# zhuzhui-2000/mobilesuperresolution

Measured on AMD Instinct MI355X. Metric: HR megapixels/sec (WDSR-B x4, 48x48 LR patches), full training step, higher is better.
Workload: dtype bf16; 1 GPU; WDSR-B x4, 16 blocks / 24 units, 48x48 LR patches, batch 32 per GPU, fwd+L1+bwd+Adam; global_batch=32, parallelism=dp1

## Files before the change

include/sr_hotpath.h:

```cpp
#ifndef SR_HOTPATH_H
#define SR_HOTPATH_H
#include <stddef.h>
#include <stdint.h>

#ifdef __cplusplus
extern "C" {
#endif

typedef void* sr_stream_t;

#define SR_DTYPE_F32 0
#define SR_DTYPE_BF16 1

int sr_abi_version(void);

int sr_wdsr_block_fwd(const void* x, void* y, const void* wblob, const float* cinit,
                      int N, int H, int W, int F, int dtype, sr_stream_t stream);

int sr_wdsr_block2_fwd(const void* x, void* ya, void* yb, const void* wblob_a, const void* wblob_b,
                       const float* cinit_a, const float* cinit_b, void* tsave_a, void* tsave_b, int N, int H, int W,
                       int F, int dtype, sr_stream_t stream);

int sr_wdsr_block2_bwd_data(const void* xa, const void* xb, const void* dyb, void* dxb, void* dxa,
                            const void* wblob_a, const void* wblob_b, const float* cinit_a, const float* cinit_b,
// ... 154 lines not shown
typedef struct { const int* idx; void* out; long src_off, src_stride; int n, reps, as_float; } sr_pack_seg_t;
typedef struct { const float* partial; const int* sidx; const int* dst; long dst_off, dst_stride, slab; int wgs, n, reps; } sr_unpack_seg_t;
int sr_param_pack(const float* flat, float* src, const int* chan_tab, int n_chan, const int* bias_tab, const float* bias_const,
                  int n_bias, const sr_pack_seg_t* segs, int nseg, int dtype, sr_stream_t stream);
int sr_param_grads(const float* flat, float* dsrc, float* gflat, const int* chan_tab, int n_chan, const int* bias_tab,
                   int n_bias, const sr_unpack_seg_t* segs, int nseg, sr_stream_t stream);

typedef struct {
  int F, NB, R, dtype, N, H, W;
  float mean;
  const float* flat; float* gflat;
  const int* chan_tab; int n_chan;
  const int* bias_tab; const float* bias_const; int n_bias;
  float* src; float* dsrc;
  long src_head_off, src_body_off, src_body_stride, src_tail_off;
  const int* idx_head; int n_idx_head;
  const int* idx_body; int n_idx_body;
  const int* idx_cinit; int n_idx_cinit;
  const int* idx_tail; int n_idx_tail;
  void* blob_head; void* blob_body; float* cinit_body; void* blob_tail;
  float* part_a; float* part_b; float* part_tail; float* part_head;
  int wgs_body, wgs_tail, wgs_head;
  int slab_a, slab_b, slab_tail, slab_head;
  const int* ga_sidx; const int* ga_dst; int n_ga;
  const int* gb_sidx; const int* gb_dst; int n_gb;
  const int* gt_sidx; const int* gt_dst; int n_gt;
  const int* gh_sidx; const int* gh_dst; int n_gh;
  const float* x; void* acts; void* grads; float* out; const float* dout;
  void* tsave; void* dtsave;
  const float* hr; int loss_kind; float loss_gscale; float* loss_part;
  int nb_split, chan_split, bias_split;
  int adam_in_wn_bwd;
  int one_block32;
} sr_wdsr_net_t;

#define SR_NET_SAVE_ACTS 1
#define SR_NET_WEIGHTS_PACKED 2
#define SR_NET_PACK_ONLY 4
#define SR_NET_SKIP_TAIL 8
int sr_wdsr_net_forward(const sr_wdsr_net_t* net, int flags, sr_stream_t stream);
int sr_wdsr_net_backward(const sr_wdsr_net_t* net, sr_stream_t stream);
int sr_wdsr_net_backward_part(const sr_wdsr_net_t* net, int part, sr_stream_t stream);

int sr_pixel_shuffle(const float* in, float* out, int N, int C, int H, int W, int r, int inverse, sr_stream_t stream);

int sr_tail_bwd_loss(const float* sr, const float* hr, int loss_kind, float gscale, float* loss_part, const void* feat,
                     const float* x_nchw, float mean, const void* wblob, void* dfeat, float* partial, int wgs, int N, int H,
                     int W, int F, int R, int dtype, sr_stream_t stream);

int sr_tail_train(const float* hr, int loss_kind, float gscale, float* loss_part, const void* feat, const float* x_nchw, float mean,
                  const void* wblob, void* dfeat, float* partial, int wgs, int N, int H, int W, int F, int R, int dtype,
                  sr_stream_t stream);

typedef struct { float w_lerp, beta2, one_minus_beta2, bc2_sqrt, eps, neg_step_size; } sr_adam_t;
int sr_adam_step(float* param, const float* grad, float* exp_avg, float* exp_avg_sq, long n, const sr_adam_t* a,
                 const float* loss_part, int n_loss, float loss_scale, float* loss_out, sr_stream_t stream);
int sr_loss_value(const float* loss_part, int n_loss, float loss_scale, float* loss_out, sr_stream_t stream);
int sr_scale_by(void* y, const void* x, long n, const float* scale, int dtype, sr_stream_t stream);
int sr_wdsr_net_train_step(const sr_wdsr_net_t* net, float* exp_avg, float* exp_avg_sq, long n_params, const sr_adam_t* a,
                           float loss_scale, float* loss_out, sr_stream_t stream);

int sr_conv7_fwd(const void* x, const void* wpacked, const float* bias, void* y, int N, int H, int W, int CIN, int COUT, int relu,
                 int out_f32, sr_stream_t stream);

int sr_probe_mfma_bf16(const void* a_frag, const void* b_frag, float* acc_out, sr_stream_t stream);
int sr_probe_mfma_f32(const float* a_frag, const float* b_frag, float* acc_out, sr_stream_t stream);
int sr_probe_tr_read(const void* img_bf16, int n_elems, const int* lane_elem_off, void* out_bf16x4,
                     sr_stream_t stream);
int sr_probe_copy(const void* src, void* dst, size_t n_bytes, sr_stream_t stream);
int sr_probe_launch_floor(void* out, int gx, int gy, int threads, int lds_bytes, int reps, sr_stream_t stream);
int sr_probe_launch_floor_graph(void* out, int gx, int gy, int threads, int lds_bytes, int reps, int iters,
                                float* us_per_launch, float* host_us_per_graph );
// ... 7 lines not shown
```

mobilesuperresolution_amd/_lib.py:

```python
from __future__ import annotations

import ctypes
import os
from ctypes import c_int, c_size_t, c_void_p

import torch

_HERE = os.path.dirname(os.path.abspath(__file__))
LIB_PATH = os.environ.get("SR_HOTPATH_LIB_PATH") or os.path.join(
    _HERE, "libsr_hotpath_dbg.so" if os.environ.get("SR_HOTPATH_DEBUG_LIB") == "1" else "libsr_hotpath.so")
ABI_VERSION = 19
DTYPE_CODE = {torch.float32: 0, torch.bfloat16: 1}
_HOT_DTYPES = {"fp32": torch.float32, "float32": torch.float32, "bf16": torch.bfloat16, "bfloat16": torch.bfloat16}


def hot_dtype(name=None) -> torch.dtype:
    name = name or os.environ.get("SR_HOT_DTYPE", "fp32")
    return name if isinstance(name, torch.dtype) else _HOT_DTYPES[str(name).lower()]


_P, _I, _Z, _L, _F = c_void_p, c_int, c_size_t, ctypes.c_long, ctypes.c_float
SIGNATURES = {
    "sr_abi_version": ([], _I),
    "sr_wdsr_block_fwd": ([_P, _P, _P, _P, _I, _I, _I, _I, _I, _P], _I),
    "sr_wdsr_block2_fwd": ([_P] * 9 + [_I] * 5 + [_P], _I),
    "sr_wdsr_fwd_rs": ([_P] * 9 + [_I] * 6 + [_P], _I),
    "sr_conv7_fwd": ([_P] * 4 + [_I] * 7 + [_P], _I),
    "sr_wdsr_fwd_rs_repeat": ([_P] * 9 + [_I] * 7 + [_P], _I),
    "sr_wdsr_block_wgrad_saved": ([_P] * 8 + [_I] * 7 + [_L] * 5 + [_P], _I),
    "sr_wdsr_block2_bwd_data": ([_P] * 11 + [_I] * 5 + [_P], _I),
    "sr_wdsr_block2_fwd_repeat": ([_P] * 7 + [_I] * 6 + [_P], _I),
    "sr_probe_launch_floor": ([_P, _I, _I, _I, _I, _I, _P], _I),
    "sr_probe_launch_floor_graph": ([_P, _I, _I, _I, _I, _I, _I, _P, _P], _I),
    "sr_debug_set_stamps": ([_P, _L], _I),
    "sr_c3_trunk_fwd": ([_P] * 6 + [_I] * 7 + [_L, _P], _I),
    "sr_c3_trunk_bwd": ([_P] * 11 + [_I] * 8 + [_L, _P], _I),
    "sr_c64_trunk_fwd": ([_P] * 7 + [_I] * 7 + [_L, _P], _I),
    "sr_c64_recon_fwd": ([_P, _P, _I, _P, _L, _P, _P, _P, _P, _P, _P, _P, _L] + [_I] * 5 + [_P], _I),
    "sr_mv_recon_fwd": ([_P, _P, _I, _P, _L, _L, _P, _P, _L, _L, _P] + [_I] * 5 + [_P], _I),
    "sr_mv_recon_bwd": ([_P, _P, _P, _P, _L, _L, _P, _P, _P, _P, _I, _P] + [_I] * 6 + [_P], _I),
    "sr_mv_recon_slab": ([], _I),
    "sr_tail_bwd": ([_P, _P, _P, _F, _P, _P, _P] + [_I] * 7 + [_P], _I),
    "sr_nas_dw_wgrad": ([_P, _P, _P, _P, _I, _I, _I, _I, _I, _I, _P], _I),
    "sr_wdsr_block_fwd_repeat": ([_P, _P, _P, _P, _I, _I, _I, _I, _I, _I, _P], _I),
# ... 31 lines not shown
    "sr_scale_by": ([_P, _P, _L, _P, _I, _P], _I),
    "sr_wdsr_net_train_step": ([_P, _P, _P, _L, _P, _F, _P, _P], _I),
    "sr_wdsr_net_forward": ([_P, _I, _P], _I),
    "sr_wdsr_net_backward": ([_P, _P], _I),
    "sr_wdsr_net_backward_part": ([_P, _I, _P], _I),
    "sr_probe_mfma_bf16": ([_P, _P, _P, _P], _I),
    "sr_probe_mfma_f32": ([_P, _P, _P, _P], _I),
    "sr_probe_tr_read": ([_P, _I, _P, _P, _P], _I),
    "sr_probe_copy": ([_P, _P, _Z, _P], _I),
    "sr_rm_block_fwd": ([_P] * 5 + [_I] * 6 + [_P], _I),
    "sr_rm_block_bwd_data": ([_P] * 4 + [_I] * 6 + [_P], _I),
    "sr_rm_wgrad": ([_P] * 4 + [_I] * 8 + [_P], _I),
    "sr_rm_tail_fwd": ([_P] * 3 + [_I] * 7 + [_P], _I),
    "sr_rm_unshuffle": ([_P, _P] + [_I] * 5 + [_P], _I),
    "sr_rm_tail_bwd_data": ([_P] * 3 + [_I] * 7 + [_P], _I),
}

class WdsrNet(ctypes.Structure):
    _fields_ = (
        [(n, _I) for n in ("F", "NB", "R", "dtype", "N", "H", "W")] + [("mean", _F)] +
        [("flat", _P), ("gflat", _P), ("chan_tab", _P), ("n_chan", _I),
         ("bias_tab", _P), ("bias_const", _P), ("n_bias", _I), ("src", _P), ("dsrc", _P)] +
        [(n, _L) for n in ("src_head_off", "src_body_off", "src_body_stride", "src_tail_off")] +
        [("idx_head", _P), ("n_idx_head", _I), ("idx_body", _P), ("n_idx_body", _I),
         ("idx_cinit", _P), ("n_idx_cinit", _I), ("idx_tail", _P), ("n_idx_tail", _I),
         ("blob_head", _P), ("blob_body", _P), ("cinit_body", _P), ("blob_tail", _P),
         ("part_a", _P), ("part_b", _P), ("part_tail", _P), ("part_head", _P)] +
        [(n, _I) for n in ("wgs_body", "wgs_tail", "wgs_head", "slab_a", "slab_b", "slab_tail", "slab_head")] +
        [("ga_sidx", _P), ("ga_dst", _P), ("n_ga", _I), ("gb_sidx", _P), ("gb_dst", _P), ("n_gb", _I),
         ("gt_sidx", _P), ("gt_dst", _P), ("n_gt", _I), ("gh_sidx", _P), ("gh_dst", _P), ("n_gh", _I),
         ("x", _P), ("acts", _P), ("grads", _P), ("out", _P), ("dout", _P), ("tsave", _P), ("dtsave", _P),
         ("hr", _P), ("loss_kind", _I), ("loss_gscale", _F), ("loss_part", _P),
         ("nb_split", _I), ("chan_split", _I), ("bias_split", _I), ("adam_in_wn_bwd", _I),
         ("one_block32", _I)])


class C3Warp(ctypes.Structure):
    _fields_ = [("frame", _P), ("frame_bs", _L), ("state", _P), ("flow", _P), ("flow_bs", _L), ("flow_bound", _P),
                ("dstate", _P), ("dflow", _P), ("dflow_bs", _L), ("x0_save", _P)]


class C3Unpack(ctypes.Structure):
    _fields_ = [("sidx0", _P), ("dst0", _P), ("n0", _I), ("sidx1", _P), ("dst1", _P), ("n1", _I), ("gflat", _P)]


class PackSeg(ctypes.Structure):
    _fields_ = [("idx", _P), ("out", _P), ("src_off", _L), ("src_stride", _L), ("n", _I), ("reps", _I), ("as_float", _I)]


class UnpackSeg(ctypes.Structure):
    _fields_ = [("partial", _P), ("sidx", _P), ("dst", _P), ("dst_off", _L), ("dst_stride", _L), ("slab", _L), ("wgs", _I),
                ("n", _I), ("reps", _I)]


class AdamScalars(ctypes.Structure):
    _fields_ = [(n, _F) for n in ("w_lerp", "beta2", "one_minus_beta2", "bc2_sqrt", "eps", "neg_step_size")]


_lib = None


class HotpathError(RuntimeError):
    pass


def _declare(lib):
    for name, (args, res) in SIGNATURES.items():
# ... 92 lines not shown
```

mobilesuperresolution_amd/csrc/sr_abi.hip:

```cpp
#include <algorithm>
#include "../../include/sr_hotpath.h"
#include "wdsr_block.h"
#include "wdsr_fwd_rs.h"
#include "wdsr_fwd_stream.h"
#include "wdsr_bwd_rs.h"
#include "wdsr_bwd_pair_lds.h"
#include "wdsr_wgrad_rs.h"
#include "wdsr_ends.h"
#include "wdsr_prep.h"
#include "conv3x3.h"
#include "conv64.h"
#include "vsr_recon.h"
#include "mv_recon.h"
#include "spynet_conv.h"
#include "nas_block.h"
#include "nas_dw_lc.h"
#include "nas_bwd_fused.h"
#include "flow_warp.h"
#include "metrics.h"
#include "patches.h"
#include "clips.h"
#include "train_step.h"
#include "pixel_shuffle.h"
#include "result_block.h"

extern "C" int sr_abi_version(void) { return 19; }

namespace {

template <int F_, int E_, int L_>
struct WdsrDimsOf {
  static constexpr int F = F_, E = E_, L = L_;
  typedef BlockCfg<F_, E_, L_> Cfg;
};
template <int F> struct WdsrDims;
template <> struct WdsrDims<24> : WdsrDimsOf<24, 144, 20> {};
template <> struct WdsrDims<32> : WdsrDimsOf<32, 192, 26> {};

template <typename Fn>
int dispatch_f(int F, Fn&& fn) {
  if (F == 24) return fn(WdsrDims<24>{});
  if (F == 32) return fn(WdsrDims<32>{});
  return -1;
}
template <typename Fn>
int dispatch_ft(int F, int dtype, Fn&& fn) {
  return dispatch_f(F, [&](auto d) {
    if (dtype == SR_DTYPE_BF16) return fn(d, __bf16{});
    if (dtype == SR_DTYPE_F32) return fn(d, float{});
    return -1;
  });
}

struct Tiles { int x, y; };
template <typename C = WdsrDims<24>::Cfg>
Tiles block_tiles(int H, int W) {
  return Tiles{(W + C::TW - 1) / C::TW, (H + C::TH - 1) / C::TH};
}

// ... 948 lines not shown
    else if (F == 32) hipLaunchKernelGGL((nas_dw_wgrad3_kernel<32>), dim3(wgs), dim3(768), 0, st, (const __bf16*)yin, (const __bf16*)GZ, dwp, partial, N, H, W, tx, tpi, vs);
    else return -1;
    SR_HIP_CHECK_LAUNCH();
    return 0;
  }
#define CALL(T, F_) { typedef NasCfg<F_> C; const int tx = (W + C::TW - 1) / C::TW, tpi = tx * ((H + C::TH - 1) / C::TH); \
    hipLaunchKernelGGL((nas_dw_wgrad_kernel<T, F_>), dim3(wgs, 3), dim3(768), 0, st, (const T*)yin, (const T*)GZ, dwp, partial, N, H, W, tx, tpi, vs); }
  SR_NAS_DISPATCH_F32(CALL)
#undef CALL
  SR_HIP_CHECK_LAUNCH();
  return 0;
}

namespace {
template <typename T> int net_pack(const sr_wdsr_net_t* n, hipStream_t st) {
  const int cb = (n->n_chan + 3) / 4, bb = (n->n_bias + 255) / 256;
  hipLaunchKernelGGL(wn_src_kernel, dim3(cb + bb), dim3(256), 0, st, n->flat, n->src, (const int4*)n->chan_tab,
                     n->n_chan, n->bias_tab, n->bias_const, n->n_bias, cb);
  PackSegs ps;
  ps.nseg = 4;
  int blk = 0;
  auto add = [&](int k, const int* idx, void* out, long off, long stride, int cnt, int reps, int as_float) {
    ps.s[k] = PackSeg{idx, out, off, stride, cnt, reps, as_float, blk};
    blk += reps * ((cnt + 255) / 256);
  };
  add(0, n->idx_head, n->blob_head, n->src_head_off, 0, n->n_idx_head, 1, 0);
  add(1, n->idx_body, n->blob_body, n->src_body_off, n->src_body_stride, n->n_idx_body, n->NB, 0);
  add(2, n->idx_cinit, n->cinit_body, n->src_body_off, n->src_body_stride, n->n_idx_cinit, n->NB, 1);
  add(3, n->idx_tail, n->blob_tail, n->src_tail_off, 0, n->n_idx_tail, 1, 0);
  hipLaunchKernelGGL((pack_all_kernel<T>), dim3(blk), dim3(256), 0, st, n->src, ps);
  SR_HIP_CHECK_LAUNCH();
  return 0;
}
}

static bool net_saves_side_images(const sr_wdsr_net_t* n, bool backward) {
  return (n->F == 24 || n->F == 32) && n->dtype == SR_DTYPE_BF16 && n->tsave && (!backward || n->dtsave);
}
static long net_tiles(const sr_wdsr_net_t* n) {
  const Tiles t = block_tiles(n->H, n->W);
  return (long)n->N * t.x * t.y;
}
static bool net_uses_pairs(const sr_wdsr_net_t* n) {
  return n->dtype == SR_DTYPE_BF16 && net_tiles(n) <= 384 && (n->F == 24 || (n->F == 32 && !n->one_block32));
}
static bool net_step_fuses_tail(const sr_wdsr_net_t* n) {
  return n->dtype == SR_DTYPE_BF16 && n->R == 4 && (n->F == 24 || n->F == 32) && n->hr && n->N <= 65535;
}
static size_t side_image_bytes(const sr_wdsr_net_t* n) {
  typedef WdsrDims<24>::Cfg C;
  const Tiles t = block_tiles<C>(n->H, n->W);
  const int lp = n->F == 24 ? C::LP : WdsrDims<32>::Cfg::LP;
  return (size_t)n->N * ((size_t)t.x * t.y) * C::TH * C::TW * lp * 2;
}
struct NetView {
  const sr_wdsr_net_t* n;
  bool keeps_side;
  size_t esz = n->dtype == SR_DTYPE_BF16 ? 2 : 4;
  size_t act_bytes = (size_t)n->N * n->H * n->W * n->F * esz, blob_bytes = (size_t)n->n_idx_body * esz;
  size_t side_bytes = side_image_bytes(n);
  char* act(int i) const { return (char*)n->acts + (size_t)i * act_bytes; }
  char* grad(int i) const { return (char*)n->grads + (size_t)i * act_bytes; }
  char* blob(int i) const { return (char*)n->blob_body + (size_t)i * blob_bytes; }
  const float* cinit(int i) const { return n->cinit_body + (size_t)i * n->n_idx_cinit; }
  char* tsave(int i) const { return keeps_side ? (char*)n->tsave + (size_t)i * side_bytes : nullptr; }
  char* dtsave(int i) const { return keeps_side ? (char*)n->dtsave + (size_t)i * side_bytes : nullptr; }
};

extern "C" int sr_wdsr_net_forward(const sr_wdsr_net_t* n, int flags, sr_stream_t stream) {
  if (!n || !n->flat || !n->src) return -2;
  if (!(flags & SR_NET_PACK_ONLY) && (!n->x || !n->acts || !n->out)) return -2;
  hipStream_t st = (hipStream_t)stream;
  const int save_acts = flags & SR_NET_SAVE_ACTS;
  int rc = 0;
  if (!(flags & SR_NET_WEIGHTS_PACKED)) rc = n->dtype == SR_DTYPE_BF16 ? net_pack<__bf16>(n, st) : net_pack<float>(n, st);
  if (rc || (flags & SR_NET_PACK_ONLY)) return rc;
  const NetView v{n, save_acts && net_saves_side_images(n, false)};
  char* acts = v.act(0);
  if ((rc = sr_head_fwd(n->x, acts, n->blob_head, n->mean, n->N, n->H, n->W, n->F, n->dtype, stream))) return rc;
  char* cur = acts;
  const bool pairs = net_uses_pairs(n) || (n->F == 24 && n->dtype == SR_DTYPE_BF16 &&
                                           ((!save_acts && net_tiles(n) >= 768) || fwd_stream_applies(n->N, n->H, n->W)));
  for (int i = 0, nb; i < n->NB; i += nb) {
    nb = pairs && i + 1 < n->NB ? 2 : 1;
    char* nxt = save_acts ? v.act(i + nb) : (cur == acts ? v.act(1) : acts);
    if (nb == 2)
      rc = sr_wdsr_block2_fwd(cur, save_acts ? v.act(i + 1) : nullptr, nxt, v.blob(i), v.blob(i + 1), v.cinit(i), v.cinit(i + 1),
                              v.tsave(i), v.tsave(i + 1), n->N, n->H, n->W, n->F, n->dtype, stream);
    else if (pairs)
      rc = sr_wdsr_fwd_rs(cur, nullptr, nxt, v.blob(i), nullptr, v.cinit(i), nullptr, v.tsave(i), nullptr, 1, n->N, n->H, n->W, n->F,
                          n->dtype, stream);
    else if (v.keeps_side)
      rc = dispatch_f(n->F, [&](auto d) {
        return launch_block_fwd<__bf16, decltype(d)::F>(cur, nxt, v.blob(i), v.cinit(i), n->N, n->H, n->W, st, v.tsave(i));
      });
    else
      rc = sr_wdsr_block_fwd(cur, nxt, v.blob(i), v.cinit(i), n->N, n->H, n->W, n->F, n->dtype, stream);
    if (rc) return rc;
    cur = nxt;
  }
  if (flags & SR_NET_SKIP_TAIL) return 0;
  return sr_tail_fwd(cur, n->x, n->out, n->blob_tail, n->mean, n->N, n->H, n->W, n->F, n->R, n->dtype, stream);
}

namespace {
struct FusedAdam { float* m; float* v; AdamArgs a; const float* loss_part; int n_loss; float loss_scale; float* loss_out; };
}
static int net_backward_part_impl(const sr_wdsr_net_t* n, int part, sr_stream_t stream, const FusedAdam* fa, bool tail_train = false) {
  if (!n || !n->flat || !n->gflat || !n->dsrc || !n->x || !n->acts || !n->grads || part < 0 || part > 2) return -2;
  if (tail_train && (part != 0 || !n->hr)) return -2;
  if (part != 2 && (n->hr ? ((!n->out && !tail_train) || !n->loss_part || (n->loss_kind != 1 && n->loss_kind != 2)) : !n->dout)) return -2;
  hipStream_t st = (hipStream_t)stream;
// ... 620 lines not shown
```

mobilesuperresolution_amd/csrc/wdsr_ends.h:

```cpp
#pragma once
#include "wdsr_block.h"

template <int F_, int R_>
struct EndsCfg {
  static constexpr int F = F_, R = R_;
  static constexpr int CO = 3 * R * R, NT = (CO + 31) / 32, COP = (CO + 7) / 8 * 8, CC = COP / 8, FC = F / 8;
  static constexpr int KST = (9 * FC + 15 + 1) / 2, KSTB = (9 * CC + 1) / 2;
  static constexpr int TH = 12, TW = 24, HW = TW + 2, HH = TH + 2, NPXH = HW * HH, NPXH_PAD = (NPXH + 31) / 32 * 32;
  static constexpr int NPT_O = (TH / 4) * (TW / 8), NPXC = TH * TW;
  static constexpr int FT_ELEMS = (NPXH_PAD + 2) * F;
  static constexpr int DC_ELEMS = (NPXH_PAD + 2) * COP;
  static constexpr int DCC_ELEMS = (NPXC + 2) * COP;
  static constexpr int DYC_ELEMS = (NPXC + 2) * F;
  template <int P> struct Img {
    static constexpr int IW = TW + 2 * P, IH = TH + 2 * P, NPI = IW * IH, ELEMS = (NPI + 8) * 4;
  };
  static constexpr int TAIL_TILES = 14 * NT;
};

template <typename T> SR_DEV typename FragOf<T>::type lds_chunk_half(const T* img, int off) {
  typedef typename FragOf<T>::half_type HalfT;
  const HalfT lo = *reinterpret_cast<const HalfT*>(img + off);
  const HalfT hi = *reinterpret_cast<const HalfT*>(img + off + 4);
  typename FragOf<T>::type f;
// ... 142 lines not shown
              v[b][j] = loss_grad<LOSS>(v[b][j], h[j], li.gscale, term);
              if (core && lsum) *lsum += term;
            }
          }
        }
      }
    }
#pragma unroll
    for (int b = 0; b < BATCH; ++b) {
      const int idx = tid + (b0 + b) * NTHREADS;
      if (b0 + b < ITER && idx < TOTAL) {
        const int p = idx / ROWS, cr = idx - p * ROWS;
        const int c = cr / R, si = cr - c * R;
        T* d = DC + p * E::COP + c * R * R + si * R;
        if constexpr (R == 4) {
          typename FragOf<T>::half_type hv;
          hv[0] = (T)v[b][0]; hv[1] = (T)v[b][1]; hv[2] = (T)v[b][2]; hv[3] = (T)v[b][3];
          *reinterpret_cast<typename FragOf<T>::half_type*>(d) = hv;
        } else {
#pragma unroll
          for (int j = 0; j < R; ++j) d[j] = (T)v[b][j];
        }
      }
    }
  }
  if constexpr (E::COP > E::CO) {
    for (int idx = tid; idx < NPX * (E::COP - E::CO); idx += NTHREADS) {
      const int p = idx / (E::COP - E::CO), k = idx - p * (E::COP - E::CO);
      DC[p * E::COP + E::CO + k] = (T)0.f;
    }
  }
}

template <typename T, int F>
__global__ __launch_bounds__(256) void sr_head_fwd_kernel(const float* __restrict__ ximg, T* __restrict__ y,
                                                          const T* __restrict__ wblob, float mean, int H, int W,
                                                          int tiles_x) {
  typedef EndsCfg<F, 4> E;
  typedef typename E::template Img<1> I;
  typedef typename FragOf<T>::half_type HalfT;
  __shared__ __attribute__((aligned(16))) T XI[I::ELEMS];
  const int tid = threadIdx.x, lane = tid & 63, wave = tid >> 6, r = lane & 31, hh = lane >> 5;
  const int n = blockIdx.y, tile = blockIdx.x;
  const int ty0 = (tile / tiles_x) * E::TH, tx0 = (tile % tiles_x) * E::TW;
  stage_img<T, E, 1>(XI, ximg + (size_t)n * 3 * H * W, mean, H, W, ty0, tx0, tid);
  __syncthreads();
  for (int ot = wave; ot < E::NPT_O; ot += 4) {
    const int oy = (ot / (E::TW / 8)) * 4 + (r >> 3), ox = (ot % (E::TW / 8)) * 8 + (r & 7);
    f32x16 acc = zero16();
#pragma unroll
    for (int s = 0; s < 3; ++s) {
      const int q = 2 * s + hh, ky = q >> 1, m = q & 1;
      acc = mma16<T>(load_wfrag<T>(wblob, s, lane), lds_chunk_half<T>(XI, ((oy + ky) * I::IW + ox + 2 * m) * 4), acc);
    }
    const int Y = ty0 + oy, X = tx0 + ox;
    if (Y < H && X < W) {
      T* yo = y + (((size_t)n * H + Y) * W + X) * F;
#pragma unroll
      for (int g = 0; g < E::FC; ++g) stream_store(reinterpret_cast<HalfT*>(yo + g * 8 + hh * 4), acc_group<T>(acc, g));
    }
  }
}

constexpr int SR_TAIL_FWD_THREADS = 512;
template <typename T, int F, int R>
__global__ __launch_bounds__(SR_TAIL_FWD_THREADS) void sr_tail_fwd_kernel(const T* __restrict__ feat, const float* __restrict__ ximg,
                                                          float* __restrict__ out, const T* __restrict__ wblob,
                                                          float mean, int H, int W, int tiles_x) {
  typedef EndsCfg<F, R> E;
  typedef typename E::template Img<2> I;
  typedef typename FragOf<T>::type FragT;
  __shared__ __attribute__((aligned(16))) T smem[E::FT_ELEMS + I::ELEMS];
  T* const FT = smem;
  constexpr int XI0 = E::FT_ELEMS;
  const int tid = threadIdx.x, lane = tid & 63, wave = tid >> 6, r = lane & 31, hh = lane >> 5;
  const int n = blockIdx.y, tile = blockIdx.x;
  const int ty0 = (tile / tiles_x) * E::TH, tx0 = (tile % tiles_x) * E::TW;
  stage_halo<T, E, F, SR_TAIL_FWD_THREADS>(FT, feat + (size_t)n * H * W * F, H, W, ty0, tx0, tid);
  stage_img<T, E, 2, SR_TAIL_FWD_THREADS>(smem + XI0, ximg + (size_t)n * 3 * H * W, mean, H, W, ty0, tx0, tid);
  __syncthreads();
  constexpr bool HOIST = (sizeof(T) == 2) && (E::NT * E::KST <= 42);
  const T* const wblob0 = wblob;
  for (int ot = wave; ot < E::NPT_O; ot += SR_TAIL_FWD_THREADS / 64) {
    wblob = weights_for_tile<HOIST>(wblob0);
    const int oy = (ot / (E::TW / 8)) * 4 + (r >> 3), ox = (ot % (E::TW / 8)) * 8 + (r & 7);
    const int hbase = oy * E::HW + ox;
    f32x16 acc[E::NT];
#pragma unroll
    for (int ti = 0; ti < E::NT; ++ti) acc[ti] = zero16();
#pragma unroll
    for (int s = 0; s < E::KST; ++s) {
      const int q = 2 * s + hh;
      FragT b;
      if (2 * s + 1 < 9 * E::FC) {
// ... 533 lines not shown
```

mobilesuperresolution_amd/layout.py:

```python
from __future__ import annotations

from collections import OrderedDict
from dataclasses import dataclass
from functools import lru_cache

import numpy as np

from . import packing as P


@dataclass(frozen=True)
class ConvSpec:
    name: str
    cout: int
    cin: int
    k: int


class WDSRLayout:
    def __init__(self, F: int, NB: int, R: int):
        self.F, self.NB, self.R = F, NB, R
        E, L = int(F * 6), int(F * 0.84)
        self.E, self.L = E, L
        CO = 3 * R * R
# ... 63 lines not shown
            base = self.src_body_off + i * ob["size"]
            ones.append(base + ob["one"])
            zeros.append(base + ob["zero"])
        self.src_ones, self.src_zeros = np.asarray(ones), np.asarray(zeros)

        bt_ = P.block_tables(F, E, L)
        et_ = P.ends_tables(F, R)
        self.idx_head = et_["head"].astype(np.int32)
        self.idx_tail = et_["tail"].astype(np.int32)
        self.idx_body = bt_["w"].astype(np.int32)
        self.idx_cinit = bt_["cinit"].astype(np.int32)

        gt = P.block_grad_tables(F, E, L)
        n_w1, n_w2, n_w3 = E * F, L * E, F * L * 9
        ga, gb = gt["a"], gt["b"]
        dst_a = np.concatenate([ob["w1"] + np.arange(n_w1), ob["w2"] + np.arange(n_w2),
                                ob["b1"] + np.arange(E), ob["b2"] + np.arange(L)])
        dst_b = np.concatenate([ob["w3"] + np.arange(n_w3), ob["b3"] + np.arange(F)])
        def by_slab(sidx, dst):
            o = np.argsort(sidx, kind="stable")
            return sidx[o].astype(np.int32), dst[o].astype(np.int32)
        self.ga = by_slab(ga, dst_a)
        self.gb = by_slab(gb, dst_b)
        self.slab_a, self.slab_b = gt["a_size"], gt["b_size"]
        ge = P.ends_grad_tables(F, R)
        n_t = CO * F * 9 + CO * 75 + CO
        dst_t = np.concatenate([ot["wt"] + np.arange(CO * F * 9), ot["ws"] + np.arange(CO * 75),
                                ot["b"] + np.arange(CO)])
        assert ge["tail"].size == n_t
        self.gt = by_slab(ge["tail"], dst_t)
        dst_h = np.concatenate([oh["wh"] + np.arange(F * 27), oh["b"] + np.arange(F)])
        self.gh = by_slab(ge["head"], dst_h)
        self.slab_tail, self.slab_head = ge["tail_size"], ge["head_size"]


    def split_at(self, nb_split: int):
        per_block = sum(c.cout for c in self.convs if c.name.startswith("body.0."))
        head_rows = next(c.cout for c in self.convs if c.name == "head")
        first = min(off for name, (off, _) in self.entries.items() if name.startswith(f"body.{nb_split}."))
        return first, head_rows + nb_split * per_block, head_rows + nb_split * per_block


@lru_cache(maxsize=None)
def get_layout(F: int, NB: int, R: int) -> WDSRLayout:
    return WDSRLayout(F, NB, R)
```

mobilesuperresolution_amd/models/basic_wdsr_b.py:

```python
from __future__ import annotations

import ctypes
import math
import os
from collections import OrderedDict

import numpy as np
import torch
import torch.nn as nn

from .. import _lib as L
from ..layout import get_layout

__all__ = ["BASIC_MODEL"]


class _DeviceState:

    def __init__(self, model: "BASIC_MODEL", device: torch.device):
        lay = model.layout
        t = lambda a: torch.from_numpy(np.ascontiguousarray(a)).to(device)
        f32 = lambda n: torch.empty(n, dtype=torch.float32, device=device)
        self.chan_tab, self.bias_tab = t(lay.chan_tab), t(lay.bias_tab)
        bc = lay.bias_const.copy()
# ... 20 lines not shown
        self.loss_part = torch.zeros(self.wgs_tail, dtype=torch.float32, device=device)
        n = L.WdsrNet()
        n.F, n.NB, n.R, n.dtype, n.mean = lay.F, lay.NB, lay.R, L.DTYPE_CODE[dt], model.image_mean
        n.chan_tab, n.n_chan = self.chan_tab.data_ptr(), lay.chan_tab.shape[0]
        n.bias_tab, n.bias_const, n.n_bias = self.bias_tab.data_ptr(), self.bias_const.data_ptr(), lay.bias_tab.shape[0]
        n.src, n.dsrc = self.src.data_ptr(), self.dsrc.data_ptr()
        n.src_head_off, n.src_body_off = lay.src_head_off, lay.src_body_off
        n.src_body_stride, n.src_tail_off = lay.src_body_stride, lay.src_tail_off
        for k in ("head", "body", "cinit", "tail"):
            setattr(n, "idx_" + k, self.idx[k].data_ptr())
            setattr(n, "n_idx_" + k, self.idx[k].numel())
        n.blob_head, n.blob_body = self.blob_head.data_ptr(), self.blob_body.data_ptr()
        n.cinit_body, n.blob_tail = self.cinit_body.data_ptr(), self.blob_tail.data_ptr()
        n.part_a, n.part_b = self.part_a.data_ptr(), self.part_b.data_ptr()
        n.part_tail, n.part_head = self.part_tail.data_ptr(), self.part_head.data_ptr()
        n.wgs_body, n.wgs_tail, n.wgs_head = self.wgs_body, self.wgs_tail, self.wgs_head
        n.slab_a, n.slab_b, n.slab_tail, n.slab_head = lay.slab_a, lay.slab_b, lay.slab_tail, lay.slab_head
        for k in ("ga", "gb", "gt", "gh"):
            setattr(n, k + "_sidx", self.g[k][0].data_ptr())
            setattr(n, k + "_dst", self.g[k][1].data_ptr())
            setattr(n, "n_" + k, self.g[k][0].numel())
        n.loss_part = self.loss_part.data_ptr()
        ct, bt = lay.chan_tab, lay.bias_tab
        cover = np.zeros(int(model.flat.numel()), dtype=np.int32)
        for v_off, g_off, K, _dst in ct:
            cover[v_off:v_off + K] += 1
            cover[g_off] += 1
        for a_, b_, _d in bt:
            cover[a_] += 1
            if b_ >= 0:
                cover[b_] += 1
        n.adam_in_wn_bwd = int(bool((cover == 1).all()))
        n.one_block32 = int(model.one_block32)
        if model.nb_split:
            _, n.chan_split, n.bias_split = lay.split_at(model.nb_split)
            n.nb_split = model.nb_split
        self.net = n

    def call_struct(self) -> "L.WdsrNet":
        return L.WdsrNet.from_buffer_copy(self.net)

    def call_net(self, x, flat, acts, out=None, dout=None, grads=None, gflat=None, side=None, dtsave=None, hr=None,
                 kind=0, gscale=0.0) -> "L.WdsrNet":
        net = self.call_struct()
        net.N, net.H, net.W = x.shape[0], x.shape[2], x.shape[3]
        net.flat, net.x, net.acts = flat.data_ptr(), x.data_ptr(), acts.data_ptr()
        if out is not None:
            net.out = out.data_ptr()
        if dout is not None:
            net.dout = dout.data_ptr()
        if grads is not None:
            net.grads, net.gflat = grads.data_ptr(), gflat.data_ptr()
        if side is not None:
            net.tsave = side.data_ptr()
        if dtsave is not None:
            net.dtsave = dtsave.data_ptr()
        if hr is not None:
            net.hr, net.loss_kind, net.loss_gscale = hr.data_ptr(), kind, gscale
        return net

    def ensure_packed(self, net, key, sp):
        if self.packed_key != key:
            _launch_net("sr_wdsr_net_forward", net, 4, sp)
            self.packed_key = key


# ... 458 lines not shown
```

Baseline: 3547 HR-Mpix/s.

## Fuse weight-norm packing and head convolution into one prologue kernel

Replaces the separate weight-norm pack step and head forward launch with a single prologue kernel. Some blocks compute per-channel norms and write the packed head, body, cinit and tail weights, while the head-conv blocks rebuild their own head weights in LDS and run the head convolution right away. This removes a launch and the dependency between packing and the head conv. In exchange it adds precomputed code and row tables, and the head blocks do redundant norm computations.

After: 3445 HR-Mpix/s. -2.9%, worse.

```diff
diff --git a/include/sr_hotpath.h b/include/sr_hotpath.h
--- a/include/sr_hotpath.h
+++ b/include/sr_hotpath.h
@@ -210,12 +210,16 @@
   int nb_split, chan_split, bias_split;
   int adam_in_wn_bwd;
   int one_block32;
+  const int* pro_tab;
+  int pro_code_off[4], pro_rows_off[4], pro_chan0[4], pro_bias0[4];
+  int pro_row_stride, pro_chunk;
 } sr_wdsr_net_t;
 
 #define SR_NET_SAVE_ACTS 1
 #define SR_NET_WEIGHTS_PACKED 2
 #define SR_NET_PACK_ONLY 4
 #define SR_NET_SKIP_TAIL 8
+#define SR_NET_SPLIT_PROLOGUE 16
 int sr_wdsr_net_forward(const sr_wdsr_net_t* net, int flags, sr_stream_t stream);
 int sr_wdsr_net_backward(const sr_wdsr_net_t* net, sr_stream_t stream);
 int sr_wdsr_net_backward_part(const sr_wdsr_net_t* net, int part, sr_stream_t stream);
diff --git a/mobilesuperresolution_amd/_lib.py b/mobilesuperresolution_amd/_lib.py
--- a/mobilesuperresolution_amd/_lib.py
+++ b/mobilesuperresolution_amd/_lib.py
@@ -9,7 +9,7 @@
 _HERE = os.path.dirname(os.path.abspath(__file__))
 LIB_PATH = os.environ.get("SR_HOTPATH_LIB_PATH") or os.path.join(
     _HERE, "libsr_hotpath_dbg.so" if os.environ.get("SR_HOTPATH_DEBUG_LIB") == "1" else "libsr_hotpath.so")
-ABI_VERSION = 19
+ABI_VERSION = 20
 DTYPE_CODE = {torch.float32: 0, torch.bfloat16: 1}
 _HOT_DTYPES = {"fp32": torch.float32, "float32": torch.float32, "bf16": torch.bfloat16, "bfloat16": torch.bfloat16}
 
@@ -107,7 +107,9 @@
          ("x", _P), ("acts", _P), ("grads", _P), ("out", _P), ("dout", _P), ("tsave", _P), ("dtsave", _P),
          ("hr", _P), ("loss_kind", _I), ("loss_gscale", _F), ("loss_part", _P),
          ("nb_split", _I), ("chan_split", _I), ("bias_split", _I), ("adam_in_wn_bwd", _I),
-         ("one_block32", _I)])
+         ("one_block32", _I),
+         ("pro_tab", _P), ("pro_code_off", _I * 4), ("pro_rows_off", _I * 4), ("pro_chan0", _I * 4), ("pro_bias0", _I * 4),
+         ("pro_row_stride", _I), ("pro_chunk", _I)])
 
 
 class C3Warp(ctypes.Structure):
diff --git a/mobilesuperresolution_amd/csrc/sr_abi.hip b/mobilesuperresolution_amd/csrc/sr_abi.hip
--- a/mobilesuperresolution_amd/csrc/sr_abi.hip
+++ b/mobilesuperresolution_amd/csrc/sr_abi.hip
@@ -8,6 +8,7 @@
 #include "wdsr_wgrad_rs.h"
 #include "wdsr_ends.h"
 #include "wdsr_prep.h"
+#include "wdsr_prologue.h"
 #include "conv3x3.h"
 #include "conv64.h"
 #include "vsr_recon.h"
@@ -24,7 +25,7 @@
 #include "pixel_shuffle.h"
 #include "result_block.h"
 
-extern "C" int sr_abi_version(void) { return 19; }
+extern "C" int sr_abi_version(void) { return 20; }
 
 namespace {
 
@@ -1039,6 +1040,40 @@
   SR_HIP_CHECK_LAUNCH();
   return 0;
 }
+template <typename T, int F> int net_prologue(const sr_wdsr_net_t* n, void* acts0, hipStream_t st) {
+  typedef EndsCfg<F, 4> E;
+  if (!n->pro_tab || n->pro_chunk != PRO_CHUNK || n->n_idx_head != 3 * 512 || n->F != F) return -2;
+  ProSegs ps;
+  ps.nseg = 4;
+  int blk = 0;
+  auto add = [&](int k, void* out, int cnt, int reps, int as_float) {
+    ps.s[k] = ProSeg{n->pro_tab + n->pro_code_off[k], n->pro_tab + n->pro_rows_off[k], out, cnt, reps, as_float, blk, n->pro_chan0[k],
+                     n->pro_bias0[k], n->pro_row_stride};
+    blk += reps * ((cnt + PRO_CHUNK - 1) / PRO_CHUNK);
+  };
+  add(0, n->blob_head, n->n_idx_head, 1, 0);
+  add(1, n->blob_body, n->n_idx_body, n->NB, 0);
+  add(2, n->cinit_body, n->n_idx_cinit, n->NB, 1);
+  add(3, n->blob_tail, n->n_idx_tail, 1, 0);
+  ProHead hd{n->x, acts0, n->mean, n->H, n->W, 0, 0, 0};
+  if (acts0) {
+    hd.tiles_x = (n->W + E::TW - 1) / E::TW;
+    hd.tiles = hd.tiles_x * ((n->H + E::TH - 1) / E::TH);
+    const long hb = (long)n->N * hd.tiles;
+    if (n->N <= 0 || n->H <= 0 || n->W <= 0 || hb + blk > 0x7fffffffL) return -2;
+    hd.blocks = (int)hb;
+  }
+  const ProTabs tb{(const int4*)n->chan_tab, n->bias_tab, n->bias_const};
+  hipLaunchKernelGGL((sr_net_prologue_kernel<T, F>), dim3(hd.blocks + blk), dim3(256), 0, st, n->flat, tb, ps, hd);
+  SR_HIP_CHECK_LAUNCH();
+  return 0;
+}
+int net_prologue_dispatch(const sr_wdsr_net_t* n, void* acts0, hipStream_t st) {
+  const int F = n->F, dtype = n->dtype;
+#define CALL(T, F_) return net_prologue<T, F_>(n, acts0, st);
+  SR_DISPATCH_TF(CALL)
+#undef CALL
+}
 }
 
 static bool net_saves_side_images(const sr_wdsr_net_t* n, bool backward) {
@@ -1080,11 +1115,18 @@
   hipStream_t st = (hipStream_t)stream;
   const int save_acts = flags & SR_NET_SAVE_ACTS;
   int rc = 0;
-  if (!(flags & SR_NET_WEIGHTS_PACKED)) rc = n->dtype == SR_DTYPE_BF16 ? net_pack<__bf16>(n, st) : net_pack<float>(n, st);
+  const NetView v{n, save_acts && net_saves_side_images(n, false)};
+  char* acts = (flags & SR_NET_PACK_ONLY) ? nullptr : v.act(0);
+  bool head_done = false;
+  if (!(flags & SR_NET_WEIGHTS_PACKED)) {
+    if (flags & SR_NET_SPLIT_PROLOGUE) rc = n->dtype == SR_DTYPE_BF16 ? net_pack<__bf16>(n, st) : net_pack<float>(n, st);
+    else {
+      rc = net_prologue_dispatch(n, acts, st);
+      head_done = true;
+    }
+  }
   if (rc || (flags & SR_NET_PACK_ONLY)) return rc;
-  const NetView v{n, save_acts && net_saves_side_images(n, false)};
-  char* acts = v.act(0);
-  if ((rc = sr_head_fwd(n->x, acts, n->blob_head, n->mean, n->N, n->H, n->W, n->F, n->dtype, stream))) return rc;
+  if (!head_done && (rc = sr_head_fwd(n->x, acts, n->blob_head, n->mean, n->N, n->H, n->W, n->F, n->dtype, stream))) return rc;
   char* cur = acts;
   const bool pairs = net_uses_pairs(n) || (n->F == 24 && n->dtype == SR_DTYPE_BF16 &&
                                            ((!save_acts && net_tiles(n) >= 768) || fwd_stream_applies(n->N, n->H, n->W)));
diff --git a/mobilesuperresolution_amd/csrc/wdsr_ends.h b/mobilesuperresolution_amd/csrc/wdsr_ends.h
--- a/mobilesuperresolution_amd/csrc/wdsr_ends.h
+++ b/mobilesuperresolution_amd/csrc/wdsr_ends.h
@@ -198,34 +198,44 @@
   }
 }
 
+template <typename T, int F, typename WS>
+SR_DEV void head_fwd_tile(const T* XI, const WS& wsrc, T* __restrict__ y, int n, int H, int W, int ty0, int tx0, int lane, int wave) {
+  typedef EndsCfg<F, 4> E;
+  typedef typename E::template Img<1> I;
+  typedef typename FragOf<T>::half_type HalfT;
+  const int r = lane & 31, hh = lane >> 5;
+  for (int ot = wave; ot < E::NPT_O; ot += 4) {
+    const int oy = (ot / (E::TW / 8)) * 4 + (r >> 3), ox = (ot % (E::TW / 8)) * 8 + (r & 7);
+    f32x16 acc = zero16();
+#pragma unroll
+    for (int s = 0; s < 3; ++s) {
+      const int q = 2 * s + hh, ky = q >> 1, m = q & 1;
+      acc = mma16<T>(wsrc.get(s, lane), lds_chunk_half<T>(XI, ((oy + ky) * I::IW + ox + 2 * m) * 4), acc);
+    }
+    const int Y = ty0 + oy, X = tx0 + ox;
+    if (Y < H && X < W) {
+      T* yo = y + (((size_t)n * H + Y) * W + X) * F;
+#pragma unroll
+      for (int g = 0; g < E::FC; ++g) stream_store(reinterpret_cast<HalfT*>(yo + g * 8 + hh * 4), acc_group<T>(acc, g));
+    }
+  }
+}
+
 template <typename T, int F>
 __global__ __launch_bounds__(256) void sr_head_fwd_kernel(const float* __restrict__ ximg, T* __restrict__ y,
                                                           const T* __restrict__ wblob, float mean, int H, int W,
                                                           int tiles_x) {
   typedef EndsCfg<F, 4> E;
   typedef typename E::template Img<1> I;
-  typedef typename FragOf<T>::half_type HalfT;
   __shared__ __attribute__((aligned(16))) T XI[I::ELEMS];
-  const int tid = threadIdx.x, lane = tid & 63, wave = tid >> 6, r = lane & 31, hh = lane >> 5;
+  const int tid = threadIdx.x, lane = tid & 63, wave = tid >> 6;
   const int n = blockIdx.y, tile = blockIdx.x;
   const int ty0 = (tile / tiles_x) * E::TH, tx0 = (tile % tiles_x) * E::TW;
   stage_img<T, E, 1>(XI, ximg + (size_t)n * 3 * H * W, mean, H, W, ty0, tx0, tid);
   __syncthreads();
-  for (int ot = wave; ot < E::NPT_O; ot += 4) {
-    const int oy = (ot / (E::TW / 8)) * 4 + (r >> 3), ox = (ot % (E::TW / 8)) * 8 + (r & 7);
-    f32x16 acc = zero16();
-#pragma unroll
-    for (int s = 0; s < 3; ++s) {
-      const int q = 2 * s + hh, ky = q >> 1, m = q & 1;
-      acc = mma16<T>(load_wfrag<T>(wblob, s, lane), lds_chunk_half<T>(XI, ((oy + ky) * I::IW + ox + 2 * m) * 4), acc);
-    }
-    const int Y = ty0 + oy, X = tx0 + ox;
-    if (Y < H && X < W) {
-      T* yo = y + (((size_t)n * H + Y) * W + X) * F;
-#pragma unroll
-      for (int g = 0; g < E::FC; ++g) stream_store(reinterpret_cast<HalfT*>(yo + g * 8 + hh * 4), acc_group<T>(acc, g));
-    }
-  }
+  WSrc<T, false> wsrc;
+  wsrc.p0 = wsrc.p = wblob;
+  head_fwd_tile<T, F>(XI, wsrc, y, n, H, W, ty0, tx0, lane, wave);
 }
 
 constexpr int SR_TAIL_FWD_THREADS = 512;
diff --git a/mobilesuperresolution_amd/csrc/wdsr_prologue.h b/mobilesuperresolution_amd/csrc/wdsr_prologue.h
--- /dev/null
+++ b/mobilesuperresolution_amd/csrc/wdsr_prologue.h
@@ -0,0 +1,122 @@
+#pragma once
+#include "wdsr_ends.h"
+#include "wdsr_prep.h"
+
+constexpr int PRO_CHUNK = 512;
+constexpr int PRO_EPT = PRO_CHUNK / 256;
+constexpr int PRO_MAXR = 64;
+constexpr int PRO_ROWS = 256;
+constexpr int PRO_B = 4, PRO_KI = 5;
+
+struct ProSeg { const int* code; const int* rows; void* out; int n, reps, as_float, block0, chan0, bias0, row_stride; };
+struct ProSegs { ProSeg s[4]; int nseg; };
+struct ProHead { const float* x; void* y; float mean; int H, W, tiles_x, tiles, blocks; };
+struct ProTabs { const int4* chan_tab; const int* bias_tab; const float* bias_const; };
+
+SR_DEV void pro_scales(const float* __restrict__ flat, const int4* __restrict__ chan_tab, const int* __restrict__ rows, int nrows,
+                       float* sc, int* vo, int lane, int wave) {
+  int myrow = 0;
+  int4 myt = make_int4(0, 0, 0, 0);
+  float myg = 0.f;
+  if (lane < nrows) {
+    myrow = rows ? rows[lane] : lane;
+    myt = chan_tab[myrow];
+    myg = flat[myt.y];
+  }
+  for (int s0 = wave * PRO_B; s0 < nrows; s0 += 4 * PRO_B) {
+    float a[PRO_B][PRO_KI];
+    int K[PRO_B], vof[PRO_B];
+#pragma unroll
+    for (int b = 0; b < PRO_B; ++b) {
+      const int s = s0 + b;
+      vof[b] = __shfl(myt.x, s & 63);
+      K[b] = s < nrows ? __shfl(myt.z, s & 63) : 0;
+#pragma unroll
+      for (int i = 0; i < PRO_KI; ++i) {
+        const int k = lane + 64 * i;
+        a[b][i] = k < K[b] ? flat[vof[b] + k] : 0.f;
+      }
+    }
+#pragma unroll
+    for (int b = 0; b < PRO_B; ++b) {
+      const int s = s0 + b;
+      const float* v = flat + vof[b];
+      float ss = 0.f;
+#pragma unroll
+      for (int i = 0; i < PRO_KI; ++i) ss = __builtin_fmaf(a[b][i], a[b][i], ss);
+      for (int k = lane + 64 * PRO_KI; k < K[b]; k += 64) { const float q = v[k]; ss = __builtin_fmaf(q, q, ss); }
+      ss = wave_sum(ss);
+      const float scale = __shfl(myg, s & 63) / sqrtf(ss);
+      const int row = __shfl(myrow, s & 63);
+      if (s < nrows && lane == 0) { sc[row] = scale; vo[row] = vof[b]; }
+    }
+  }
+}
+
+SR_DEV float pro_value(int code, const float* __restrict__ flat, const float* sc, const int* vo, const ProTabs& tb, int bias_row0) {
+  if (code >= 0) {
+    const int row = code >> 10, k = code & 1023;
+    return flat[vo[row] + k] * sc[row];
+  }
+  if (code >= -2) return code == -1 ? 0.f : 1.f;
+  const int i = bias_row0 + (-3 - code);
+  const int a = tb.bias_tab[3 * i], b = tb.bias_tab[3 * i + 1];
+  return flat[a] + (b >= 0 ? flat[b] : 0.f) + tb.bias_const[i];
+}
+
+template <typename T, int F>
+__global__ __launch_bounds__(256) void sr_net_prologue_kernel(const float* __restrict__ flat, ProTabs tb, ProSegs segs, ProHead hd) {
+  typedef EndsCfg<F, 4> E;
+  typedef typename E::template Img<1> I;
+  constexpr int NHEAD = 3 * 512;
+  __shared__ __attribute__((aligned(16))) T XI[I::ELEMS];
+  __shared__ __attribute__((aligned(16))) T WB[NHEAD];
+  __shared__ float sc[PRO_ROWS];
+  __shared__ int vo[PRO_ROWS];
+  const int tid = threadIdx.x, lane = tid & 63, wave = tid >> 6;
+  if ((int)blockIdx.x < hd.blocks) {
+    const ProSeg& sg = segs.s[0];
+    const int n = blockIdx.x / hd.tiles, tile = blockIdx.x - n * hd.tiles;
+    const int ty0 = (tile / hd.tiles_x) * E::TH, tx0 = (tile % hd.tiles_x) * E::TW;
+    int code[NHEAD / 256];
+#pragma unroll
+    for (int e = 0; e < NHEAD / 256; ++e) code[e] = sg.code[tid + 256 * e];
+    stage_img<T, E, 1>(XI, hd.x + (size_t)n * 3 * hd.H * hd.W, hd.mean, hd.H, hd.W, ty0, tx0, tid);
+    pro_scales(flat, tb.chan_tab + sg.chan0, nullptr, F, sc, vo, lane, wave);
+    __syncthreads();
+#pragma unroll
+    for (int e = 0; e < NHEAD / 256; ++e) WB[tid + 256 * e] = (T)pro_value(code[e], flat, sc, vo, tb, sg.bias0);
+    __syncthreads();
+    WSrc<T, true> wsrc;
+    wsrc.p = WB;
+    head_fwd_tile<T, F>(XI, wsrc, reinterpret_cast<T*>(hd.y), n, hd.H, hd.W, ty0, tx0, lane, wave);
+    return;
+  }
+  const int pb = blockIdx.x - hd.blocks;
+  int k = 0;
+#pragma unroll
+  for (int i = 1; i < 4; ++i) if (i < segs.nseg && pb >= segs.s[i].block0) k = i;
+  const ProSeg sg = segs.s[k];
+  const int per_rep = (sg.n + PRO_CHUNK - 1) / PRO_CHUNK;
+  const int b = pb - sg.block0, rep = b / per_rep, chunk = b - rep * per_rep;
+  if (rep >= sg.reps) return;
+  int code[PRO_EPT];
+#pragma unroll
+  for (int e = 0; e < PRO_EPT; ++e) {
+    const int i = chunk * PRO_CHUNK + 256 * e + tid;
+    code[e] = i < sg.n ? sg.code[i] : -1;
+  }
+  const int* rows = sg.rows + chunk * (PRO_MAXR + 1);
+  pro_scales(flat, tb.chan_tab + sg.chan0 + rep * sg.row_stride, rows + 1, rows[0], sc, vo, lane, wave);
+  __syncthreads();
+  const int bias_row0 = sg.bias0 + rep * sg.row_stride;
+#pragma unroll
+  for (int e = 0; e < PRO_EPT; ++e) {
+    const int i = chunk * PRO_CHUNK + 256 * e + tid;
+    if (i < sg.n) {
+      const float v = pro_value(code[e], flat, sc, vo, tb, bias_row0);
+      if (sg.as_float) reinterpret_cast<float*>(sg.out)[(size_t)rep * sg.n + i] = v;
+      else reinterpret_cast<T*>(sg.out)[(size_t)rep * sg.n + i] = (T)v;
+    }
+  }
+}
diff --git a/mobilesuperresolution_amd/layout.py b/mobilesuperresolution_amd/layout.py
--- a/mobilesuperresolution_amd/layout.py
+++ b/mobilesuperresolution_amd/layout.py
@@ -119,7 +119,56 @@
         dst_h = np.concatenate([oh["wh"] + np.arange(F * 27), oh["b"] + np.arange(F)])
         self.gh = by_slab(ge["head"], dst_h)
         self.slab_tail, self.slab_head = ge["tail_size"], ge["head_size"]
+        self._prologue_tables()
 
+    PRO_CHUNK, PRO_MAXR, PRO_ROWS = 512, 64, 256
+    PRO_ZERO, PRO_ONE, PRO_BIAS = -1, -2, -3
+
+    def _prologue_tables(self):
+        NB, per = self.NB, self.E + self.L + self.F
+        kind = np.zeros(self.src_total, dtype=np.int8)
+        krow = np.zeros(self.src_total, dtype=np.int64)
+        kk = np.zeros(self.src_total, dtype=np.int64)
+        for c, (_v, _g, K, dst) in enumerate(self.chan_tab):
+            assert K < 1024 and not kind[dst:dst + K].any()
+            kind[dst:dst + K], krow[dst:dst + K], kk[dst:dst + K] = 1, c, np.arange(K)
+        for i, (_a, _b, dst) in enumerate(self.bias_tab):
+            assert kind[dst] == 0
+            kind[dst], krow[dst] = 2, i
+        kind[self.src_zeros], kind[self.src_ones] = 3, 4
+        assert kind.all(), "every src entry is a weight, a bias or a constant"
+        head_rows = self.F
+        self.pro_chan0 = [0, head_rows, head_rows, head_rows + NB * per]
+        self.pro_bias0 = [0, head_rows, head_rows, self.n_plain_bias]
+        self.pro_row_stride = per
+        assert self.n_plain_bias == head_rows + NB * per and per <= self.PRO_ROWS
+        segs = (("head", self.idx_head, self.src_head_off), ("body", self.idx_body, self.src_body_off),
+                ("cinit", self.idx_cinit, self.src_body_off), ("tail", self.idx_tail, self.src_tail_off))
+        self.pro_code, self.pro_rows = {}, {}
+        for s, (name, idx, off) in enumerate(segs):
+            pos = off + idx.astype(np.int64)
+            kd, row, k = kind[pos], krow[pos], kk[pos]
+            wrow, brow = row - self.pro_chan0[s], row - self.pro_bias0[s]
+            assert ((wrow >= 0) & (wrow < self.PRO_ROWS))[kd == 1].all() and (brow >= 0)[kd == 2].all()
+            code = np.select([kd == 1, kd == 2, kd == 3], [(wrow << 10) | k, self.PRO_BIAS - brow, self.PRO_ZERO], self.PRO_ONE)
+            nchunk = (idx.size + self.PRO_CHUNK - 1) // self.PRO_CHUNK
+            rows = np.zeros((nchunk, 1 + self.PRO_MAXR), dtype=np.int32)
+            for c in range(nchunk):
+                sl = slice(c * self.PRO_CHUNK, (c + 1) * self.PRO_CHUNK)
+                u = np.unique(wrow[sl][kd[sl] == 1])
+                assert u.size <= self.PRO_MAXR, (name, c, u.size)
+                rows[c, 0], rows[c, 1:1 + u.size] = u.size, u
+            self.pro_code[name], self.pro_rows[name] = code.astype(np.int32), rows
+        parts, self.pro_code_off, self.pro_rows_off, n = [], [], [], 0
+        for name, _i, _o in segs:
+            self.pro_code_off.append(n)
+            parts.append(self.pro_code[name])
+            n += parts[-1].size
+        for name, _i, _o in segs:
+            self.pro_rows_off.append(n)
+            parts.append(self.pro_rows[name].reshape(-1))
+            n += parts[-1].size
+        self.pro_tab = np.concatenate(parts).astype(np.int32)
 
     def split_at(self, nb_split: int):
         per_block = sum(c.cout for c in self.convs if c.name.startswith("body.0."))
diff --git a/mobilesuperresolution_amd/models/basic_wdsr_b.py b/mobilesuperresolution_amd/models/basic_wdsr_b.py
--- a/mobilesuperresolution_amd/models/basic_wdsr_b.py
+++ b/mobilesuperresolution_amd/models/basic_wdsr_b.py
@@ -76,6 +76,12 @@
                 cover[b_] += 1
         n.adam_in_wn_bwd = int(bool((cover == 1).all()))
         n.one_block32 = int(model.one_block32)
+        self.pro_tab = t(lay.pro_tab)
+        n.pro_tab = self.pro_tab.data_ptr()
+        for k in range(4):
+            n.pro_code_off[k], n.pro_rows_off[k] = lay.pro_code_off[k], lay.pro_rows_off[k]
+            n.pro_chan0[k], n.pro_bias0[k] = lay.pro_chan0[k], lay.pro_bias0[k]
+        n.pro_row_stride, n.pro_chunk = lay.pro_row_stride, lay.PRO_CHUNK
         if model.nb_split:
             _, n.chan_split, n.bias_split = lay.split_at(model.nb_split)
             n.nb_split = model.nb_split
```
